# AwesomePeiweiPan/Droid-SLAM_Reserch

Measured on AMD Instinct MI355X. Metric: BA update iters/sec (2000-edge equivalents; 256 keyframes, 48x64), higher is better.
Workload: dtype f32; 1 GPU; 256-keyframe / 2000-edge global BA, 48x64, t0=1, lm=1e-5 ep=1e-2 (BASELINE configs[2]); edges_total=2000, solve=fp64 dense Cholesky on device, chol_failed=False

## Files before the change

droid-slam_reserch_amd/csrc/api.hip:

```cpp
#include <hip/hip_runtime.h>
#include <stdarg.h>
#include <stdio.h>

#include <map>
#include <mutex>

#include "../../include/droid_backends_hip.h"
#include "../../include/droid_test_hooks_hip.h"
#include "../../include/droid_heads_hip.h"
#include "../../include/droid_motion_encode_hip.h"
#include "../../include/droid_update_hip.h"
#include "ba_internal.hpp"
#include "graph.hpp"
#include "launchers.hpp"

using namespace droid;

static thread_local char g_err[512] = "";

static std::map<const void*, int*> g_mirror;
static std::mutex g_mirror_mu;
struct HintState { int* ptr; int tag; };
static std::map<const void*, HintState> g_hint;
static int g_hint_tag = 0;
static void hints_of(BaView& v, const void* ws, bool new_call) {
  std::lock_guard<std::mutex> lock(g_mirror_mu);
  auto it = g_hint.find(ws);
  if (it == g_hint.end()) return;
  if (new_call) it->second.tag = g_hint_tag = g_hint_tag >= (1 << 30) ? 1 : g_hint_tag + 1;
  if (it->second.tag == 0) return;
  v.hint = it->second.ptr;
  v.hint_tag = it->second.tag;
}
static int* mirror_of(const void* ws) {
  std::lock_guard<std::mutex> lock(g_mirror_mu);
  auto it = g_mirror.find(ws);
  return it == g_mirror.end() ? nullptr : it->second;
}

static int fail(int code, const char* fmt, ...) {
  va_list ap;
  va_start(ap, fmt);
  vsnprintf(g_err, sizeof(g_err), fmt, ap);
  va_end(ap);
  return code;
}

static int fail_hip(const char* where, hipError_t e) {
  return e == hipSuccess ? DROID_OK : fail(DROID_E_HIP, "%s: %s", where, hipGetErrorString(e));
}

static int check_hip(const char* where) { return fail_hip(where, hipGetLastError()); }

static bool bytes_overlap(const void* p, uint64_t p_bytes, const void* q, uint64_t q_bytes) {
  const uintptr_t a = (uintptr_t)p, b = (uintptr_t)q;
  const uintptr_t a1 = a + (p_bytes > UINTPTR_MAX - a ? UINTPTR_MAX - a : p_bytes);
  const uintptr_t b1 = b + (q_bytes > UINTPTR_MAX - b ? UINTPTR_MAX - b : q_bytes);
  return p_bytes > 0 && q_bytes > 0 && a < b1 && b < a1;
}
static uint64_t f32_bytes(uint64_t elems) { return elems > UINT64_MAX / 4 ? UINT64_MAX : elems * 4; }

// ... 434 lines not shown
  if (hints) {
    hints[0] = hints[1] = 0;
    g_hint[workspace] = HintState{hints, 0};
  }
  else g_hint.erase(workspace);
  return DROID_OK;
}

int droid_ba_attach_status_mirror(const void* workspace, int* mirror) {
  if (!workspace) return fail(DROID_E_ARG, "ba_attach_status_mirror: null %s", "workspace");
  std::lock_guard<std::mutex> lock(g_mirror_mu);
  if (mirror) g_mirror[workspace] = mirror;
  else g_mirror.erase(workspace);
  return DROID_OK;
}

int droid_test_wave_reduce32(const float* in, float* out, void* stream) {
  if (!in || !out) return fail(DROID_E_ARG, "test_wave_reduce32: null %s", "pointer");
  launch_wave_reduce32_test(in, out, (hipStream_t)stream);
  return check_hip("test_wave_reduce32");
}

int droid_test_ba_lin(const float* poses, const float* disps, const float* intrinsics, const float* disps_sens,
                      const float* targets, const float* weights, const float* eta, const int64_t* ii, const int64_t* jj,
                      int E, int nbuf, int H, int W, int M, int t0, int t1, int motion_only, int ragged, void* workspace,
                      size_t workspace_bytes, float* hpart_out, float* q_out, float* w_out, float* ebuf_out,
                      size_t* words_out, void* stream) {
  const BaDims d{E, nbuf, H, W, M, t0, t1, motion_only};
  BaView v;
  if (int rc = ba_view(v, workspace, workspace_bytes, d)) return rc;
  if (!poses || !disps || !intrinsics) return fail(DROID_E_ARG, "test_ba_lin: null %s", "state pointer");
  if (E > 0 && (!targets || !weights || !ii || !jj)) return fail(DROID_E_ARG, "test_ba_lin: null %s", "edge data");
  if (!motion_only && v.M > 0 && (!eta || !disps_sens)) return fail(DROID_E_ARG, "test_ba_lin: null %s", "eta/disps_sens");
  hipStream_t s = (hipStream_t)stream;
  const size_t words[4] = {(size_t)E * v.nch * LIN_WAVES * 32, (size_t)v.M * v.HW, (size_t)v.M * v.HW,
                           v.wide ? 6 * ((size_t)v.M + E) * v.HW : 0};
  const float* src[4] = {v.Hpart, v.Q, v.w, v.Ebuf};
  float* dst[4] = {hpart_out, q_out, w_out, ebuf_out};
  if (dst[0] || dst[1] || dst[2] || dst[3])
    launch_lin_test(v, poses, disps, intrinsics, disps_sens, targets, weights, eta, ii, jj, motion_only != 0, ragged != 0, s);
  if (words_out) {
    words_out[4] = (size_t)v.wide;
    words_out[5] = (size_t)v.zsplit;
  }
  for (int k = 0; k < 4; k++) {
    if (words_out) words_out[k] = words[k];
    if (dst[k] && words[k])
      (void)hipMemcpyAsync(dst[k], src[k], sizeof(float) * words[k], hipMemcpyDeviceToDevice, s);
  }
  return check_hip("test_ba_lin");
}

size_t droid_chol_scratch_doubles(int n) { return CholSystem::scratch_doubles(n); }

int droid_chol_solve(const double* A, const double* b, double* x, int n, double* scratch,
                     int* fail_flag, void* stream) {
  if (n <= 0 || !A || !b || !x || !scratch || !fail_flag) return fail(DROID_E_ARG, "chol_solve: bad %s", "argument");
  hipStream_t s = (hipStream_t)stream;
  const CholSystem c(scratch, n, x, fail_flag);
  launch_chol_pack(A, b, c.S, c.n, c.ld, s);
  launch_chol_solve(c, 0.0, 0.0, s, false);
  return check_hip("chol_solve");
}

int droid_frame_distance(const float* poses, const float* disps, const float* intrinsics,
                         const int64_t* ii, const int64_t* jj, int E, int nbuf, int H, int W,
                         float beta, float* dist, void* stream) {
  if (E < 0 || nbuf <= 0 || H <= 0 || W <= 0) return fail(DROID_E_ARG, "frame_distance: bad %s", "sizes");
  if (E == 0) return DROID_OK;
  if (!poses || !disps || !intrinsics || !ii || !jj || !dist) return fail(DROID_E_ARG, "frame_distance: null %s", "pointer");
  launch_frame_distance(poses, disps, intrinsics, ii, jj, E, nbuf, H, W, beta, dist, (hipStream_t)stream);
  return check_hip("frame_distance");
}

int droid_frame_distance_matrix(const float* poses, const float* disps, const float* intrinsics, int n, int nbuf,
                                int H, int W, float beta, float* dist, void* stream) {
  if (n < 0 || nbuf <= 0 || n > nbuf || H <= 0 || W <= 0) return fail(DROID_E_ARG, "frame_distance_matrix: bad %s", "sizes");
  if (n == 0) return DROID_OK;
  if (!poses || !disps || !intrinsics || !dist) return fail(DROID_E_ARG, "frame_distance_matrix: null %s", "pointer");
  launch_frame_distance_matrix(poses, disps, intrinsics, n, H, W, beta, dist, (hipStream_t)stream);
  return check_hip("frame_distance_matrix");
}

int droid_projmap(const float* poses, const float* disps, const float* intrinsics,
                  const int64_t* ii, const int64_t* jj, int E, int nbuf, int H, int W,
                  float* coords, float* valid, void* stream) {
  if (E < 0 || nbuf <= 0 || H <= 0 || W <= 0) return fail(DROID_E_ARG, "projmap: bad %s", "sizes");
  if (E == 0) return DROID_OK;
  if (!poses || !disps || !intrinsics || !ii || !jj || !coords || !valid) return fail(DROID_E_ARG, "projmap: null %s", "pointer");
  launch_projmap(poses, disps, intrinsics, ii, jj, E, nbuf, H, W, coords, valid, (hipStream_t)stream);
  return check_hip("projmap");
}

int droid_reproject_motion(const float* poses, const float* disps, const float* intrinsics, int intr_stride,
                           const int64_t* ii, const int64_t* jj, const float* target, int E, int nbuf, int H, int W,
                           float* coords, float* valid, float* motn, void* stream) {
  if (E < 0 || nbuf <= 0 || H <= 0 || W <= 0 || (intr_stride != 0 && intr_stride != 4))
    return fail(DROID_E_ARG, "reproject_motion: bad %s", "sizes");
  if (E == 0) return DROID_OK;
  if (!poses || !disps || !intrinsics || !ii || !jj || !coords || !valid) return fail(DROID_E_ARG, "reproject_motion: null %s", "pointer");
  if (motn && !target) return fail(DROID_E_ARG, "reproject_motion: motn needs %s", "target");
  launch_reproject_motion(poses, disps, intrinsics, intr_stride, ii, jj, target, E, nbuf, H, W, coords, valid, motn,
                          (hipStream_t)stream);
  return check_hip("reproject_motion");
}

// ... 374 lines not shown
```

droid-slam_reserch_amd/csrc/ba_internal.hpp:

```cpp
#pragma once
#include <hip/hip_runtime.h>
#include <stddef.h>
#include <stdint.h>

namespace droid {

constexpr int LIN_THREADS = 256;
constexpr int LIN_PPT = 2;
constexpr int LIN_CP = LIN_THREADS * LIN_PPT;
constexpr int LIN_WAVES = LIN_THREADS / 64;
constexpr int CHOL_NB = 64;
__host__ __device__ inline int chol_ld(int n) { return (n + 1 + 15) & ~15; }
__host__ __device__ inline size_t chol_flag_words(int n) { return 2 * ((size_t)(n + 1 + CHOL_NB - 1) / CHOL_NB) + 8; }
__host__ __device__ inline int chol_tile_index(int nrb, int bi, int bj) { return bj * nrb - bj * (bj - 1) / 2 + (bi - bj); }
__host__ __device__ inline size_t chol_tiles(int n) {
  const int nb = (n + CHOL_NB - 1) / CHOL_NB, nrb = (n + 1 + CHOL_NB - 1) / CHOL_NB;
  return (size_t)chol_tile_index(nrb, nb, nb);
}
__host__ __device__ inline size_t chol_mbuf_offset(int n) { return ((size_t)(n + CHOL_NB - 1) / CHOL_NB) * CHOL_NB * CHOL_NB; }
__host__ __device__ inline size_t chol_lfin_offset(int n) { return 2 * chol_mbuf_offset(n); }
__host__ __device__ inline size_t chol_ldiag_doubles(int n) { return chol_lfin_offset(n) + chol_tiles(n) * CHOL_NB * CHOL_NB; }
__host__ __device__ inline int chol_bs_pairs_grid(int nb) { return (nb + 1) / 2; }
__host__ __device__ inline int chol_bs_pairs_owner(int col) { return col / 2; }
__host__ __device__ inline int chol_bs_pairs_first(int wg) { return 2 * wg; }

__host__ __device__ inline size_t pk_colbase(int n, int J) {
  return (size_t)CHOL_NB * ((size_t)J * (size_t)(n + 1) - (size_t)CHOL_NB * (size_t)J * (size_t)(J - 1) / 2);
}
__host__ __device__ inline int pk_width(int n, int J) { return (n - CHOL_NB * J) < CHOL_NB ? (n - CHOL_NB * J) : CHOL_NB; }
__host__ __device__ inline size_t pk_total(int n) {
  if (n <= 0) return 0;
  const int nb = (n + CHOL_NB - 1) / CHOL_NB;
  return pk_colbase(n, nb - 1) + (size_t)(n + 1 - CHOL_NB * (nb - 1)) * (size_t)pk_width(n, nb - 1);
}
__host__ __device__ inline size_t pk_index(int n, int gi, int gj) {
  const int J = gj / CHOL_NB;
  return pk_colbase(n, J) + (size_t)(gi - CHOL_NB * J) * (size_t)pk_width(n, J) + (size_t)(gj - CHOL_NB * J);
}
__host__ __device__ inline unsigned pk_index32(int n, int gi, int gj) {
  const int J = gj >> 6, c0 = J << 6;
  const int w = (n - c0) < CHOL_NB ? (n - c0) : CHOL_NB;
  return (unsigned)(CHOL_NB * (J * (n + 1) - (CHOL_NB / 2) * J * (J - 1)) + (gi - c0) * w + (gj - c0));
}

enum { HDR_STATUS = 0, HDR_M = 1, HDR_CHOL_FAIL = 2, HDR_NENT = 3, HDR_NWORK = 4,
       HDR_NC1 = 5, HDR_NC2 = 6,
       HDR_WORDS = 16 };
enum { STATUS_BAD_INDEX = 1, STATUS_ETA_ROWS = 2, STATUS_CHOL_FAIL = 4, STATUS_CHOL_STALL = 8 };

struct BaView {
  int E, nbuf, H, W, HW;
  int t0, t1, P, M;
  int n, ld;
  int nch;
  int own0, own1;
  int motion_only;
  int* hdr;
  int* slot_of;
  int* kx;
  int* seg_ptr;
  int* seg_edge;
  int* cursor;
  int* ent_ptr;
  int* ent_row;
  int* ent_pose;
  int* wk_ptr;
  int* order;
  int* xtmp;
  int* cls_list;
  int* gt_ptr;
  double* Gpart;
  int s2_split;
  float* Hpart;
  float* Q;
// ... 89 lines not shown
  v.Gpart = nullptr;
  if (M > 0) {
    const int ptiles = (v.HW + 63) / 64;
    int ns = S2_WGS / M;
    v.s2_split = ns < 1 ? 1 : (ns > ptiles ? ptiles : ns);
    size_t tiles = (size_t)E * 7 / 4 + (size_t)M + 1;
    if (tiles > (size_t)28 * M) tiles = (size_t)28 * M;
    v.Gpart = static_cast<double*>(take(sizeof(double) * (tiles * v.s2_split * 256 + 64)));
  }
  v.sys = static_cast<double*>(take(sizeof(double) * ((size_t)(v.n + 1) * v.ld + 8)));
  v.psys = static_cast<double*>(take(sizeof(double) * (pk_total(v.n) + 8)));
  v.packed = 0;
  v.xsol = static_cast<double*>(take(sizeof(double) * ((size_t)v.ld + 1)));
  v.bs_flags = static_cast<int*>(take(sizeof(int) * chol_flag_words(v.n)));
  v.ldiag = static_cast<double*>(take(sizeof(double) * chol_ldiag_doubles(v.n)));
  v.dx = static_cast<float*>(take(sizeof(float) * ((size_t)v.n + 8)));
  v.ov_ready = static_cast<int*>(take(sizeof(int) * ((size_t)(v.n + 1 + CHOL_NB - 1) / CHOL_NB + 8)));
  v.pose_snap = static_cast<float*>(take(sizeof(float) * 7 * (size_t)nbuf));
  return off;
}

__host__ __device__ inline int solver_preset_words(const BaView& v) {
  return (int)((reinterpret_cast<const char*>(v.bs_flags) - reinterpret_cast<const char*>(v.xsol)) / 4 +
               (long)chol_flag_words(v.n));
}
__host__ __device__ inline int solver_preset_tiles(const BaView& v) { return v.n > 0 ? (int)chol_tiles(v.n) : 0; }

struct BaLaunchPlan {
  int zero_wgs;
  int asm_units;
  dim3 schur2;
  int sf_split;
  dim3 syrk[2], fold;
};
inline BaLaunchPlan ba_launch_plan(const BaView& v) {
  BaLaunchPlan p;
  p.zero_wgs = LIN_ZERO_WGS;
  p.asm_units = v.E > 0 ? v.E + (solver_preset_words(v) + 1023) / 1024 + solver_preset_tiles(v) : 0;
  p.schur2 = dim3(v.M + (p.asm_units + 4 * v.s2_split - 1) / (4 * v.s2_split), v.s2_split);
  const int tiles = (v.HW + SF_TP - 1) / SF_TP, ns = SF_WGS / (v.M > 0 ? v.M : 1);
  p.sf_split = ns < 1 ? 1 : (ns > tiles ? tiles : ns);
  p.syrk[0] = dim3(v.M, v.sy_ns[0], 1);
  p.syrk[1] = dim3(v.M, v.sy_ns[1], 4);
  p.fold = dim3(v.M, SY_FOLD_GROUPS, 2);
  return p;
}

struct CholSystem {
  double* S; int n, ld; double* x; int* flags; double* ldiag; int* fail;
  explicit CholSystem(const BaView& v)
      : S(v.sys), n(v.n), ld(v.ld), x(v.xsol), flags(v.bs_flags), ldiag(v.ldiag), fail(v.hdr + HDR_CHOL_FAIL) {}
  CholSystem(double* scratch, int n, double* x, int* fail);
  static size_t scratch_doubles(int n);
};

void launch_wave_reduce32_test(const float* in, float* out, hipStream_t s);
void launch_lin_test(const BaView& v, const float* poses, const float* disps, const float* intr, const float* sens,
                     const float* targets, const float* weights, const float* eta, const int64_t* ii, const int64_t* jj,
                     bool motion_only, bool ragged, hipStream_t s);
void launch_prep(const BaView& v, const int64_t* ii, const int64_t* jj, hipStream_t s);
void launch_unpack_system(const BaView& v, hipStream_t s);
void launch_build_stage(const BaView& v, const BaLaunchPlan& plan, const float* poses, const float* disps,
                        const float* intr, const float* sens, const float* targets, const float* weights,
                        const float* eta, const int64_t* ii, const int64_t* jj, bool motion_only,
                        int stage, hipStream_t s);
void launch_update(const BaView& v, float* poses, float* disps, const float* intr, const float* weights,
                   const int64_t* ii, const int64_t* jj, const double* x, float* dx_out, float* dz_out,
                   bool motion_only, hipStream_t s, int* status_mirror = nullptr);
void launch_chol_preset(const CholSystem& c, hipStream_t s);
bool launch_chol_factor(const CholSystem& c, double lm, double ep, hipStream_t s);
void launch_chol_backsolve(const CholSystem& c, bool factor_single, hipStream_t s);
void launch_chol_solve(const CholSystem& c, double lm, double ep, hipStream_t s, bool preset_done);

void launch_unpack_cols(const BaView& v, int J0, int J1, double lm, double ep, int epoch, hipStream_t s);
bool launch_chol_factor_overlap(const CholSystem& c, const int* ready, int epoch, hipStream_t s);
bool chol_overlap_available(int n);

}
```

droid-slam_reserch_amd/csrc/chol.hip:

```cpp
#include <hip/hip_runtime.h>
#include <mutex>

#include <cstdint>
#include <cstdlib>

#include "ba_internal.hpp"
#include "launchers.hpp"

namespace droid {

constexpr int NB = CHOL_NB;

#ifdef CHOL_STAMPS
__device__ unsigned long long g_chol_stamps[64 * 16];
__device__ unsigned long long g_bs_stamps[64 * 8];
__shared__ unsigned long long g_chol_lstamps[16];
extern "C" int droid_debug_chol_stamps(unsigned long long* out) {
  return (int)hipMemcpyFromSymbol(out, HIP_SYMBOL(g_chol_stamps), sizeof(unsigned long long) * 64 * 16);
}
extern "C" int droid_debug_bs_stamps(unsigned long long* out) {
  return (int)hipMemcpyFromSymbol(out, HIP_SYMBOL(g_bs_stamps), sizeof(unsigned long long) * 64 * 8);
}
#define STEP_STAMP(slot)                                                                                      \
  do { if (threadIdx.x == 0 && panel && (blockIdx.x < 2))                                                      \
// ... 583 lines not shown
      if (wave < nd) {
        const int q = p + 1 + wave;
        wave_gemm_nt16<true>(&B2[(16 * q) * LDP + 16 * p], &B2[(16 * q) * LDP + 16 * p], &Wl[WLB * p], WLP);
      } else if (solve_rows && wave < nd + 4) {
        const int g = wave - nd;
        wave_gemm_nt16<true>(&BT[(16 * g) * LDP + 16 * p], &BT[(16 * g) * LDP + 16 * p], &Wl[WLB * p], WLP);
      }
    }
    if (p == 0) TILE_STAMP(10);
    __syncthreads();
    if (p == 0) TILE_STAMP(5);
    if (PERSIST && solve_rows && wave == 4)
      chol_strip_out(S, ld, lfin_slot(Ldiag, n, bi, kp), BT, r0, c0, wk, nrows, p, (p == 3) ? &done[bi] : nullptr,
                     4 * kp + 3);
    if (p == 3) break;
    const int q = p + 1;
    if (wave == 0) {
      wave_gemm_nt16<false>(&B2[(16 * q) * LDP + 16 * q], &B2[(16 * q) * LDP + 16 * p],
                            &B2[(16 * q) * LDP + 16 * p], LDP);
      wave_potrf16(&B2[(16 * q) * LDP + 16 * q], &Wl[WLB * q], Idn, fail, diag);
      if (p == 0) TILE_STAMP(6);
    } else {
      int cnt = 0;
#pragma unroll 1
      for (int r = q; r < 4; r++)
#pragma unroll 1
        for (int s2 = q; s2 <= r; s2++) {
          if (r == q && s2 == q) continue;
          {
            const int slot = cnt % 2;
            const int owner = 1 + slot + ((1 + slot >= q) ? 1 : 0);
            if (owner == wave)
              wave_gemm_nt16<false>(&B2[(16 * r) * LDP + 16 * s2], &B2[(16 * r) * LDP + 16 * p],
                                    &B2[(16 * s2) * LDP + 16 * p], LDP);
          }
          cnt++;
        }
      const bool mine = (wave >= 5) ? (ndef > 0) : (ndef > 0 && wave == q);
      if (mine) {
        f64x4 acc = dacc[0];
        if (!PERSIST && k >= 0) strip_update_tile(acc, B0, B1, dg, q);
#pragma unroll
        for (int pp = 0; pp < 3; pp++)
          if (pp <= p) block_update16(acc, &BT[(16 * dg) * LDP + 16 * pp], &B2[(16 * q) * LDP + 16 * pp]);
        store_solve(acc, dg, q);
        dacc[0] = dacc[1];
        dacc[1] = dacc[2];
      }
    }
    __syncthreads();
    if (p == 0) TILE_STAMP(7);
  }
  TILE_STAMP(8);
  if (PERSIST && bi == kp + 1 && kp + 1 < (n + NB - 1) / NB) {
    __syncthreads();
    if (wave < 4) {
      const int g = wave;
#pragma unroll
      for (int q = 3; q >= 0; q--) {
        lds_f64* Cq = &BT[(16 * g) * LDP + 16 * q];
        f64x4 acc;
#pragma unroll
        for (int i = 0; i < 4; i++) acc[i] = Cq[(fg + 4 * i) * LDP + fr];
#pragma unroll
        for (int s2 = q + 1; s2 < 4; s2++)
#pragma unroll
          for (int kk = 0; kk < 16; kk += 4)
            acc = __builtin_amdgcn_mfma_f64_16x16x4f64(-BT[(16 * g + fr) * LDP + 16 * s2 + kk + fg],
                                                       B2[(16 * s2 + kk + fg) * LDP + 16 * q + fr], acc, 0, 0, 0);
#pragma unroll
        for (int i = 0; i < 4; i++) Cq[(fg + 4 * i) * LDP + fr] = acc[i];
        f64x4 m = {0.0, 0.0, 0.0, 0.0};
#pragma unroll
        for (int kk = 0; kk < 16; kk += 4)
          m = __builtin_amdgcn_mfma_f64_16x16x4f64(Cq[fr * LDP + kk + fg], Wl[WLB * q + (kk + fg) * WLP + fr], m, 0, 0, 0);
#pragma unroll
        for (int i = 0; i < 4; i++) Cq[(fg + 4 * i) * LDP + fr] = m[i];
      }
      gbl_f64* Mj = Ldiag + chol_mbuf_offset(n) + (size_t)kp * NB * NB;
#pragma unroll
      for (int it = 0; it < 8; it++) {
        const int u = it * 64 + lane;
        const int i = 16 * g + (u >> 5), j2 = (u & 31) * 2;
        f64x2 v = *(const lds_f64x2*)&BT[i * LDP + j2];
        if (r0 + i >= n) v = (f64x2){0.0, 0.0};
        *(gbl_f64x2*)&Mj[i * NB + j2] = v;
      }
    }
  }
  if (PERSIST && diag) {
#pragma unroll
    for (int e = t; e < 1024; e += 512) {
      const int pb = e >> 8, j = (e >> 4) & 15, kk = e & 15;
      const int br = pb == 3 ? 1 : 0, bc = pb == 3 ? 2 : pb + 1;
      B2[(16 * br + j) * LDP + 16 * bc + kk] = Wl[WLB * pb + WLP * j + kk];
    }
    __syncthreads();
  }
  if (grp == 0) {
    if (diag) {
      if (PERSIST) store_tile64(Ldiag + (size_t)kp * NB * NB, B2, NB, 0, 0, 0, NB, NB, false);
      else store_tile64(S, B2, ld, c0, c0, c0, c0 + wk, wk, true);
    }
  } else if (solve_rows && !PERSIST) {
    store_tile64(S, BT, ld, r0, c0, max(r0, c0 + wk), min(r0 + NB, nrows), wk, false);
  }
  if (!PERSIST) TILE_STAMP(9);
}

__global__ __launch_bounds__(512) void chol_step_kernel(double* __restrict__ S, int n, int ld, int k,
                                                        int* __restrict__ fail, double lm, double ep) {
  chol_tile<false>((gbl_f64*)S, n, ld, k, k + 1 + (int)blockIdx.x, k + 1 + (int)blockIdx.y, fail, lm, ep, nullptr,
                   nullptr, nullptr);
}


template <bool OV>
__device__ __attribute__((noinline)) void chol_tile_persist(double* __restrict__ S, int n, int ld, int k, int bi,
                                                            int bj, int* __restrict__ fail, double lm, double ep,
                                                            double* __restrict__ Ldiag, int* __restrict__ done,
                                                            int* __restrict__ abortf, bool coh_first, int k_last) {
  chol_tile<true, OV>((gbl_f64*)S, n, ld, k, bi, bj, fail, lm, ep, (gbl_f64*)Ldiag, done, abortf, coh_first, k_last);
}

struct CfpInput { const int* flag; int need; const gbl_f64* slot; };
__device__ __forceinline__ bool cfp_waits_for_done(int bj, int k, bool panel) { return k >= 0 && !panel && bj != k + 2; }
__device__ __forceinline__ int cfp_first_step(int bj) { return (bj == 0) ? -1 : 0; }
template <bool OV>
__device__ __forceinline__ CfpInput cfp_input(int lane, int bi, int bj, int k, bool panel, const int* done,
                                              const int* dver, const int* ready, int epoch, double* Ldiag, int n) {
  const bool flagged = cfp_waits_for_done(bj, k, panel);
  CfpInput in = {nullptr, 4 * k + 3, nullptr};
// ... 384 lines not shown
    if (B > 0 && rowb < B) {                                                                           \
      double u0 = 0.0, u1 = 0.0;                                                                       \
      _Pragma("unroll") for (int ii = 0; ii < 16; ii += 2) {                                           \
        const f64x2 xx = *(const lds_f64x2*)&DROID_LDS(xk)[16 * B + ii];                                \
        u0 = fma(Lcol[16 * B + ii], xx[0], u0);                                                        \
        u1 = fma(Lcol[16 * B + ii + 1], xx[1], u1);                                                    \
      }                                                                                                \
      z -= u0 + u1;                                                                                    \
    }
    DROID_BS_BLOCK(3)
    DROID_BS_BLOCK(2)
    DROID_BS_BLOCK(1)
    DROID_BS_BLOCK(0)
#undef DROID_BS_BLOCK
#undef DROID_BS_WTERM
#undef DROID_BS_STEP
    BS_STAMP(2);
    if (FAST && j < nb - 1) xsol -= poll_matvec(j + 1, Mc);
    if (__double_as_longlong(xsol) == BSP_SENTINEL) xsol = __longlong_as_double(0x7ff8000000000000LL);
    BS_STAMP(4);
    if (t < wj) __hip_atomic_store(&x[c0 + t], xsol, __ATOMIC_RELAXED, __HIP_MEMORY_SCOPE_AGENT);
    BS_STAMP(5);
  }
}

#ifdef CHOL_STAMPS
#define BS_STAMP_W(slot, wv) do { if (threadIdx.x == 64 * (wv) && blockIdx.x < 64) g_bs_stamps[blockIdx.x * 8 + (slot)] = wall_clock64(); } while (0)
#else
#define BS_STAMP_W(slot, wv) do { } while (0)
#endif

struct BspTileRegs { f64x2 v[4]; };
__device__ __forceinline__ BspTileRegs bsp_tile_issue(const gbl_f64* __restrict__ src, size_t pitch, int rows_valid) {
  const int t = threadIdx.x;
  BspTileRegs r;
#pragma unroll
  for (int it = 0; it < 4; it++) {
    const int idx2 = it * 512 + t, i = idx2 >> 5, j = (idx2 & 31) * 2;
    const bool ok = i < rows_valid;
    r.v[it] = *(const gbl_f64x2*)(src + (ok ? (size_t)i * pitch + j : 0));
    if (!ok) r.v[it] = (f64x2){0.0, 0.0};
  }
  return r;
}
__device__ __forceinline__ void bsp_tile_store(lds_f64* __restrict__ dst, const BspTileRegs& r) {
  const int t = threadIdx.x;
#pragma unroll
  for (int it = 0; it < 4; it++) {
    const int idx2 = it * 512 + t, i = idx2 >> 5, j = (idx2 & 31) * 2;
    *(lds_f64x2*)(&dst[i * LDP + j]) = r.v[it];
  }
}

constexpr int BSP_DC = 10 * 256;
__device__ __forceinline__ int bsp_dc_source(int e) {
  const int blk = e >> 7, i = (e & 127) >> 3, j = (e & 7) * 2;
  int br, bc;
  if (blk < 6) {
    br = blk < 1 ? 1 : (blk < 3 ? 2 : 3);
    bc = blk - br * (br - 1) / 2;
  } else {
    br = blk == 9 ? 1 : 0;
    bc = blk == 9 ? 2 : blk - 5;
  }
  return (16 * br + i) * NB + 16 * bc + j;
}

__device__ __forceinline__ void bsp_times_inverse(lds_f64* T, const lds_f64* D, int g, int lane) {
  const int fr = lane & 15, fg = lane >> 4;
#pragma unroll
  for (int q = 3; q >= 0; q--) {
    lds_f64* Cq = &T[(16 * g) * LDP + 16 * q];
    f64x4 acc;
#pragma unroll
    for (int i = 0; i < 4; i++) acc[i] = Cq[(fg + 4 * i) * LDP + fr];
#pragma unroll
    for (int s2 = q + 1; s2 < 4; s2++)
#pragma unroll
      for (int kk = 0; kk < 16; kk += 4)
        acc = __builtin_amdgcn_mfma_f64_16x16x4f64(-T[(16 * g + fr) * LDP + 16 * s2 + kk + fg],
                                                   D[(s2 * (s2 - 1) / 2 + q) * 256 + (kk + fg) * 16 + fr], acc, 0, 0, 0);
#pragma unroll
    for (int i = 0; i < 4; i++) Cq[(fg + 4 * i) * LDP + fr] = acc[i];
    f64x4 m = {0.0, 0.0, 0.0, 0.0};
#pragma unroll
    for (int kk = 0; kk < 16; kk += 4)
      m = __builtin_amdgcn_mfma_f64_16x16x4f64(Cq[fr * LDP + kk + fg], D[(6 + q) * 256 + (kk + fg) * 16 + fr], m, 0, 0, 0);
#pragma unroll
    for (int i = 0; i < 4; i++) Cq[(fg + 4 * i) * LDP + fr] = m[i];
  }
}

template <int NN>
__device__ __forceinline__ double bsp_dot(const double* col, const lds_f64* xs) {
  double a0 = 0.0, a1 = 0.0, a2 = 0.0, a3 = 0.0;
#pragma unroll
  for (int r = 0; r < NN; r += 4) {
    const f64x2 x01 = *(const lds_f64x2*)&xs[r], x23 = *(const lds_f64x2*)&xs[r + 2];
    a0 = fma(col[r + 0], x01[0], a0);
    a1 = fma(col[r + 1], x01[1], a1);
    a2 = fma(col[r + 2], x23[0], a2);
    a3 = fma(col[r + 3], x23[1], a3);
  }
  return (a0 + a1) + (a2 + a3);
}

__global__ __launch_bounds__(512) void chol_backsolve_pairs_kernel(
    double* __restrict__ S_, int n, int ld, double* __restrict__ x, int* __restrict__ err,
    const double* __restrict__ Ldiag_) {
  __shared__ double Dc[2][BSP_DC];
  __shared__ double Nt[3][NB * LDP];
  __shared__ double xs[8][NB];
  __shared__ double far_part[8][NB];
  __shared__ double near_part[8][NB];
  __shared__ double us[2][NB];
  __shared__ int dead;
  const gbl_f64* const S = (const gbl_f64*)S_;
  const gbl_f64* const Ldiag = (const gbl_f64*)Ldiag_;
  const int t = threadIdx.x, w = t >> 6, l = t & 63;
  const int nb = (n + NB - 1) / NB, G = gridDim.x, J = blockIdx.x;
  const int b = chol_bs_pairs_first(J), a = b + 1;
  const bool has_a = a < nb;
  const bool above = a + 1 < nb;
  const bool above2 = a + 2 < nb;
  const int ch = w & 1, rq = w >> 1;
  lds_f64* const xw = DROID_LDS(xs[w]);
  BS_STAMP_W(0, 0);
  if (t == 0) dead = 0;

  const int ra = (a + 1) * NB, rb = (a + 2) * NB;
  BspTileRegs t0, t1, t2;
  f64x2 dreg[5];
  if (above) {
    t1 = bsp_tile_issue(S + (size_t)ra * ld + (size_t)b * NB, ld, n - ra);
    if (above2) {
      t2 = bsp_tile_issue(S + (size_t)rb * ld + (size_t)b * NB, ld, n - rb);
      t0 = bsp_tile_issue(S + (size_t)rb * ld + (size_t)a * NB, ld, n - rb);
    }
#pragma unroll
    for (int it = 0; it < 5; it++) {
      const int idx2 = it * 512 + t, which = idx2 >= BSP_DC / 2 ? 1 : 0;
      dreg[it] = *(const gbl_f64x2*)(Ldiag + (size_t)(b + which) * NB * NB + bsp_dc_source(idx2 - which * (BSP_DC / 2)));
    }
  }

  double keep[NB];
  {
    const gbl_f64* base = Ldiag;
    int row_lo = 0, col_lo = l, row_hi = 0, used = 0;
    if (w == 4 || (w == 5 && has_a)) {
      const int pb = l >> 4;
      base = Ldiag + (size_t)(b + w - 4) * NB * NB;
      row_lo = pb == 3 ? 16 : 0;
      col_lo = 16 * (pb == 3 ? 2 : pb + 1) + (l & 15);
      used = NB;
    } else if (w == 6 && has_a) {
      base = Ldiag + chol_mbuf_offset(n) + (size_t)b * NB * NB;
      used = NB;
    } else if (ch == 1 && rq < 2 && above) {
      base = Ldiag + chol_mbuf_offset(n) + (size_t)a * NB * NB;
      row_lo = row_hi = 32 * rq;
      used = 32;
    }
#pragma unroll
    for (int i = 0; i < NB; i++) {
      keep[i] = 0.0;
      if (i < used) keep[i] = base[(size_t)((i < 16 ? row_lo : row_hi) + i) * NB + (i < 16 ? col_lo : l)];
    }
  }
  double z = 0.0;
  if ((w == 4 || (w == 5 && has_a)) && (b + w - 4) * NB + l < n) z = S[(size_t)n * ld + (b + w - 4) * NB + l];

  if (above) {
    bsp_tile_store(DROID_LDS(Nt[1]), t1);
    if (above2) {
      bsp_tile_store(DROID_LDS(Nt[2]), t2);
      bsp_tile_store(DROID_LDS(Nt[0]), t0);
    }
#pragma unroll
    for (int it = 0; it < 5; it++) *(lds_f64x2*)&DROID_LDS(Dc[0])[2 * (it * 512 + t)] = dreg[it];
    __syncthreads();
    if (w < 4) {
      bsp_times_inverse(DROID_LDS(Nt[1]), DROID_LDS(Dc[0]), w, l);
      if (above2) bsp_times_inverse(DROID_LDS(Nt[0]), DROID_LDS(Dc[1]), w, l);
    } else if (above2) {
      bsp_times_inverse(DROID_LDS(Nt[2]), DROID_LDS(Dc[0]), w - 4, l);
    }
  }
  BS_STAMP_W(1, 0);

  auto poll = [&](int gi, int lanes) -> double {
    double xv = 0.0;
    if (l < lanes && gi + l < n) {
      int spins = 0;
      while (true) {
        xv = __hip_atomic_load(&x[gi + l], __ATOMIC_RELAXED, __HIP_MEMORY_SCOPE_AGENT);
        if (__double_as_longlong(xv) != BSP_SENTINEL) break;
        if (++spins > (1 << 22)) {
          *(volatile int*)&dead = 1;
          atomicMax(err, 2);
          xv = 0.0;
          break;
        }
        __builtin_amdgcn_s_sleep(1);
      }
    }
    return xv;
  };

  double far = 0.0;
  for (int P = G - 1; P >= J + 2; P--) {
    if (*(volatile int*)&dead) break;
    const int r0 = 2 * P * NB + 32 * rq;
    const gbl_f64* col = S + (size_t)(b + ch) * NB + l;
    double Tc[32];
#pragma unroll
    for (int r = 0; r < 32; r++) {
      const int row = r0 + r;
      Tc[r] = col[(size_t)(row < n ? row : n - 1) * ld];
      if (row >= n) Tc[r] = 0.0;
    }
    const double xv = poll(r0, 32);
    if (l < 32) xw[l] = xv;
    far += bsp_dot<32>(Tc, xw);
  }
  DROID_LDS(far_part[w])[l] = far;
  BS_STAMP_W(2, 0);
  __syncthreads();
  if (dead) return;

  if (w == 4 || (w == 5 && has_a)) {
    const int c = w - 4;
    z -= (far_part[c][l] + far_part[2 + c][l]) + (far_part[4 + c][l] + far_part[6 + c][l]);
    const int rowb = l >> 4;
    double xsol = 0.0;
#define DROID_BSP_WTERM(ACC, C)                                                                         \
    asm volatile("v_fmac_f64_dpp %0, %1, %2 row_newbcast:" #C " row_mask:0xf bank_mask:0xf"             \
                 : "+v"(ACC) : "v"(z), "v"(keep[C]));
#define DROID_BSP_BLOCK(B)                                                                              \
    if (rowb == B) {                                                                                   \
// ... 183 lines not shown
  return false;
}

extern "C" int droid_debug_bs_pairs_map(int nb, int* owner) {
  for (int j = 0; j < nb; j++) owner[j] = chol_bs_pairs_owner(j);
  return chol_bs_pairs_grid(nb);
}

void launch_chol_backsolve(const CholSystem& c, bool factor_single, hipStream_t s) {
  const int nb = (c.n + NB - 1) / NB;
  if (nb >= 2 && nb <= BSP_MAX_BLOCKS) {
    CholSystem a = c;
    const double* ld_arg = factor_single ? c.ldiag : nullptr;
    void* args[] = {&a.S, &a.n, &a.ld, &a.x, &a.fail, &ld_arg};
    const bool pairs = factor_single && chol_switches().bs_pairs;
    const void* fn = pairs ? (const void*)chol_backsolve_pairs_kernel
                   : factor_single ? (const void*)chol_backsolve_persistent_kernel<true>
                                   : (const void*)chol_backsolve_persistent_kernel<false>;
    if (launch_spinning_grid(fn, pairs ? chol_bs_pairs_grid(nb) : nb, pairs ? 512 : 256, args, s,
                             chol_switches().force_bs_refusal)) return;
  }
  if (factor_single)
    hipLaunchKernelGGL(chol_ldiag_to_sys_kernel, dim3(nb), dim3(256), 0, s, c.S, c.n, c.ld, c.ldiag);
  for (int k = nb - 1; k >= 0; k--) {
    const int c0 = k * NB;
    hipLaunchKernelGGL(chol_backsolve_kernel, dim3(1 + (c0 + 255) / 256), dim3(256), 0, s, c.S, c.n,
                       c.ld, k, c.x);
  }
}

void launch_chol_preset(const CholSystem& c, hipStream_t s) {
  (void)hipMemsetAsync(c.fail, 0, sizeof(int), s);
  const size_t xbytes = sizeof(double) * (size_t)c.n, fbytes = sizeof(int) * chol_flag_words(c.n);
  const char* xb = reinterpret_cast<const char*>(c.x);
  const char* fb = reinterpret_cast<const char*>(c.flags);
  if (fb >= xb + xbytes && fb - xb <= (ptrdiff_t)(xbytes + 4096)) {
    (void)hipMemsetAsync(c.x, 0xFF, (size_t)(fb - xb) + fbytes, s);
  } else {
    (void)hipMemsetAsync(c.x, 0xFF, xbytes, s);
    (void)hipMemsetAsync(c.flags, 0xFF, fbytes, s);
  }
  (void)hipMemsetAsync(c.ldiag + chol_lfin_offset(c.n), 0xFF, sizeof(double) * chol_tiles(c.n) * NB * NB, s);
}

void launch_chol_solve(const CholSystem& c, double lm, double ep, hipStream_t s, bool preset_done) {
  if (c.n <= 0) return;
  if (!preset_done) launch_chol_preset(c, s);
  const bool single = launch_chol_factor(c, lm, ep, s);
  launch_chol_backsolve(c, single, s);
}

size_t CholSystem::scratch_doubles(int n) {
  if (n <= 0) return 0;
  return (size_t)(n + 1) * chol_ld(n) + chol_ldiag_doubles(n) + (chol_flag_words(n) + 1) / 2 + 16;
}
CholSystem::CholSystem(double* scratch, int n_, double* x_, int* fail_)
    : S(scratch), n(n_), ld(chol_ld(n_)), x(x_), fail(fail_) {
  ldiag = S + (size_t)(n + 1) * ld;
  flags = reinterpret_cast<int*>(ldiag + chol_ldiag_doubles(n));
}

__global__ void chol_pack_kernel(const double* __restrict__ A, const double* __restrict__ b,
                                 double* __restrict__ S, int n, int ld) {
  const size_t idx = (size_t)blockIdx.x * blockDim.x + threadIdx.x;
  if (idx >= (size_t)(n + 1) * ld) return;
  const int r = (int)(idx / ld), c = (int)(idx % ld);
  double val = 0.0;
  if (r < n && c < n) val = A[(size_t)r * n + c];
  else if (r == n && c < n) val = b[c];
  S[idx] = val;
}

void launch_chol_pack(const double* A, const double* b, double* S, int n, int ld, hipStream_t s) {
  const size_t tot = (size_t)(n + 1) * ld;
  hipLaunchKernelGGL(chol_pack_kernel, dim3((unsigned)((tot + 255) / 256)), dim3(256), 0, s, A, b,
                     S, n, ld);
}

}
```

droid-slam_reserch_amd/droid_backends/_lib.py:

```python
from __future__ import annotations

import ctypes
import os

_HERE = os.path.dirname(os.path.abspath(__file__))
LIB_PATH = os.environ.get("DROID_HIP_LIB") or os.path.join(_HERE, "libdroid_backends_hip.so")

ABI = {
    "droid_abi_version": ("i", ""),
    "droid_last_error": ("s", ""),
    "droid_corr_index_forward": ("i", "3p 7i p"),
    "droid_corr_index_backward": ("i", "3p 7i p"),
    "droid_corr_pyramid_forward": ("i", "P 2p 6i p"),
    "droid_corr_volume_pyramid": ("i", "3p P 7i 2l i p"),
    "droid_corr_pyramid_forward_slots": ("i", "P 3p i l 5i p"),
    "droid_corr_volume_pyramid_slots": ("i", "3p P p 7i l i p"),
    "droid_altcorr_forward": ("i", "4p 9i p"),
    "droid_altcorr_backward": ("i", "6p 8i p"),
    "droid_altcorr_pyramid_forward": ("i", "P 4p 7i p"),
    "droid_altcorr_pyramid_forward_f16": ("i", "P 4p 7i p"),
    "droid_ba_workspace_bytes": ("z", "7i"),
    "droid_ba": ("i", "9p 8i 2f i 3p z p"),
    "droid_ba_prepare": ("i", "2p 10i p z p"),
    "droid_ba_build": ("i", "9p 8i p z p"),
# ... 5 lines not shown
    "droid_ba_unpack_chunk": ("i", "9i 2f i p z p"),
    "droid_ba_solve_update_overlap": ("i", "6p 9i 3p z p"),
    "droid_ba_solve_update": ("i", "6p 7i 2f i 3p z p"),
    "droid_ba_profile_iteration": ("i", "9p 7i 2f i p z 2p"),
    "droid_ba_system": ("p", "p 7i Z"),
    "droid_ba_status": ("i", "2p 2I"),
    "droid_ba_attach_status_mirror": ("i", "2p"),
    "droid_ba_attach_launch_hints": ("i", "2p"),
    "droid_chol_solve": ("i", "3p i 3p"),
    "droid_chol_scratch_doubles": ("z", "i"),
    "droid_reproject_motion": ("i", "3p i 3p 4i 4p"),
    "droid_frame_distance": ("i", "5p 4i f 2p"),
    "droid_frame_distance_matrix": ("i", "3p 4i f 2p"),
    "droid_projmap": ("i", "5p 4i 3p"),
    "droid_iproj": ("i", "3p 3i 2p"),
    "droid_depth_filter": ("i", "5p 4i 2p"),
    "droid_proximity_workspace_bytes": ("z", "5i"),
    "droid_proximity_edges": ("i", "p 7i f 2i 2p i 2p i p i 2p z p"),
    "droid_cvx_upsample": ("i", "4p 6i p"),
    "droid_graph_mean_workspace_bytes": ("z", "2i"),
    "droid_graph_mean": ("i", "3p i l 4i 2p z p"),
    "droid_se3_unary": ("i", "2p l i p"),
    "droid_se3_mul": ("i", "p i p i p l p"),
    "droid_pose_interpolate": ("i", "2p i p i 4p"),
    "droid_point_cloud_workspace_bytes": ("z", "3i"),
    "droid_point_cloud": ("i", "6p 5i d 6p z p"),
    "droid_test_wave_reduce32": ("i", "3p"),
}
SYMBOLS = list(ABI)
ABI_UPDATE = {
    "droid_ba_inputs_workspace_bytes": ("z", "3i"),
    "droid_ba_inputs": ("i", "11p 9i f 6p i 3p i 2p z p"),
}
SYMBOLS_UPDATE = list(ABI_UPDATE)
ABI_CORR_ENCODE = {
    "droid_corr_encode_packed_bytes": ("z", ""),
    "droid_corr_encode": ("i", "P 4p i l 7i p"),
}
SYMBOLS_CORR_ENCODE = list(ABI_CORR_ENCODE)
ABI_MOTION_ENCODE = {
    "droid_motion_encode_packed_bytes": ("z", ""),
    "droid_motion_encode": ("i", "3p i 8p 5i p"),
}
SYMBOLS_MOTION_ENCODE = list(ABI_MOTION_ENCODE)
ABI_HEADS = {
    "droid_head_packed_bytes": ("z", "i"),
    "droid_update_heads": ("i", "3P 2I 5i p"),
}
SYMBOLS_HEADS = list(ABI_HEADS)
ABI_TEST = {
    "droid_test_ba_lin": ("i", "9p 9i p z 4p Z p"),
}
SYMBOLS_TEST = list(ABI_TEST)
_CTYPE = {"i": ctypes.c_int, "l": ctypes.c_int64, "z": ctypes.c_size_t, "f": ctypes.c_float, "d": ctypes.c_double,
          "p": ctypes.c_void_p, "P": ctypes.POINTER(ctypes.c_void_p), "I": ctypes.POINTER(ctypes.c_int),
          "Z": ctypes.POINTER(ctypes.c_size_t), "s": ctypes.c_char_p}


def signature(name):
    for table in (ABI, ABI_TEST, ABI_CORR_ENCODE, ABI_MOTION_ENCODE, ABI_HEADS):
        if name in table:
            break
    else:
        table = ABI_UPDATE
    res, args = table[name]
    return _CTYPE[res], [_CTYPE[run[-1]] for run in args.split() for _ in range(int(run[:-1] or 1))]


DROID_F16, DROID_F32, DROID_F64 = 0, 1, 2

_lib = None


class DroidBackendError(RuntimeError):
    pass


def load() -> ctypes.CDLL:
    global _lib
    if _lib is not None:
        return _lib
    if not os.path.exists(LIB_PATH):
        raise DroidBackendError(
            f"{LIB_PATH} is missing: build the HIP extension first "
            "(python -c 'import __graft_entry__ as g; g.build()' or droid-slam_reserch_amd/csrc/build.sh). "
            "There is no CPU fallback.")
    lib = ctypes.CDLL(LIB_PATH)
    for s in SYMBOLS + SYMBOLS_UPDATE + SYMBOLS_CORR_ENCODE + SYMBOLS_MOTION_ENCODE + SYMBOLS_HEADS + SYMBOLS_TEST:
        if not hasattr(lib, s):
            if s in SYMBOLS_TEST:
                continue
            raise DroidBackendError(f"{LIB_PATH} does not export {s}")
        fn = getattr(lib, s)
        fn.restype, fn.argtypes = signature(s)
    if lib.droid_abi_version() != 1:
        raise DroidBackendError("ABI version mismatch")
    _lib = lib
    return lib


def check(rc: int, what: str):
    if rc != 0:
        msg = load().droid_last_error().decode("utf-8", "replace")
        raise RuntimeError(f"droid_backends.{what} failed (rc={rc}): {msg}")
```

Baseline: 2086 iters/s.

## Precompute inverse-scaled off-diagonal tiles in factor for pair backsolve

The factor kernel now also writes the inverse-scaled sub-diagonal tiles for blocks two and three below the panel into new scratch buffers (N2, N3). The pair backsolve kernel loads those precomputed tiles directly. This drops its own loads of the diagonal-inverse blocks and the LDS triangular multiply by the inverse. The cost is extra scratch memory and extra MFMA work and stores in the factor tail, plus a test hook that exposes the scratch layout.

```diff
diff --git a/droid-slam_reserch_amd/csrc/api.hip b/droid-slam_reserch_amd/csrc/api.hip
--- a/droid-slam_reserch_amd/csrc/api.hip
+++ b/droid-slam_reserch_amd/csrc/api.hip
@@ -7,6 +7,7 @@
 
 #include "../../include/droid_backends_hip.h"
 #include "../../include/droid_test_hooks_hip.h"
+#include "../../include/droid_chol_hooks_hip.h"
 #include "../../include/droid_heads_hip.h"
 #include "../../include/droid_motion_encode_hip.h"
 #include "../../include/droid_update_hip.h"
@@ -547,6 +548,18 @@
 }
 
 size_t droid_chol_scratch_doubles(int n) { return CholSystem::scratch_doubles(n); }
+
+int droid_test_chol_layout(int n, int64_t* out) {
+  if (n <= 0 || !out) return fail(DROID_E_ARG, "test_chol_layout: bad %s", "argument");
+  const size_t ldiag = CholSystem::scratch_ldiag(n);
+  out[0] = chol_ld(n);
+  out[1] = (int64_t)ldiag;
+  out[2] = (int64_t)(ldiag + chol_mbuf_offset(n));
+  out[3] = (int64_t)(ldiag + chol_n2_offset(n));
+  out[4] = (int64_t)(ldiag + chol_n3_offset(n));
+  out[5] = (n + CHOL_NB - 1) / CHOL_NB;
+  return DROID_OK;
+}
 
 int droid_chol_solve(const double* A, const double* b, double* x, int n, double* scratch,
                      int* fail_flag, void* stream) {
diff --git a/droid-slam_reserch_amd/csrc/ba_internal.hpp b/droid-slam_reserch_amd/csrc/ba_internal.hpp
--- a/droid-slam_reserch_amd/csrc/ba_internal.hpp
+++ b/droid-slam_reserch_amd/csrc/ba_internal.hpp
@@ -19,7 +19,9 @@
 }
 __host__ __device__ inline size_t chol_mbuf_offset(int n) { return ((size_t)(n + CHOL_NB - 1) / CHOL_NB) * CHOL_NB * CHOL_NB; }
 __host__ __device__ inline size_t chol_lfin_offset(int n) { return 2 * chol_mbuf_offset(n); }
-__host__ __device__ inline size_t chol_ldiag_doubles(int n) { return chol_lfin_offset(n) + chol_tiles(n) * CHOL_NB * CHOL_NB; }
+__host__ __device__ inline size_t chol_n2_offset(int n) { return chol_lfin_offset(n) + chol_tiles(n) * CHOL_NB * CHOL_NB; }
+__host__ __device__ inline size_t chol_n3_offset(int n) { return chol_n2_offset(n) + chol_mbuf_offset(n); }
+__host__ __device__ inline size_t chol_ldiag_doubles(int n) { return chol_n3_offset(n) + chol_mbuf_offset(n); }
 __host__ __device__ inline int chol_bs_pairs_grid(int nb) { return (nb + 1) / 2; }
 __host__ __device__ inline int chol_bs_pairs_owner(int col) { return col / 2; }
 __host__ __device__ inline int chol_bs_pairs_first(int wg) { return 2 * wg; }
@@ -215,6 +217,7 @@
       : S(v.sys), n(v.n), ld(v.ld), x(v.xsol), flags(v.bs_flags), ldiag(v.ldiag), fail(v.hdr + HDR_CHOL_FAIL) {}
   CholSystem(double* scratch, int n, double* x, int* fail);
   static size_t scratch_doubles(int n);
+  static size_t scratch_ldiag(int n);
 };
 
 void launch_wave_reduce32_test(const float* in, float* out, hipStream_t s);
diff --git a/droid-slam_reserch_amd/csrc/chol.hip b/droid-slam_reserch_amd/csrc/chol.hip
--- a/droid-slam_reserch_amd/csrc/chol.hip
+++ b/droid-slam_reserch_amd/csrc/chol.hip
@@ -659,7 +659,10 @@
     if (p == 0) TILE_STAMP(7);
   }
   TILE_STAMP(8);
-  if (PERSIST && bi == kp + 1 && kp + 1 < (n + NB - 1) / NB) {
+  const int below = bi - kp;
+  const bool leaves_n = PERSIST && bi < (n + NB - 1) / NB &&
+                        (below == 1 || below == 2 || (below == 3 && chol_bs_pairs_first(chol_bs_pairs_owner(kp)) == kp));
+  if (leaves_n) {
     __syncthreads();
     if (wave < 4) {
       const int g = wave;
@@ -684,7 +687,8 @@
 #pragma unroll
         for (int i = 0; i < 4; i++) Cq[(fg + 4 * i) * LDP + fr] = m[i];
       }
-      gbl_f64* Mj = Ldiag + chol_mbuf_offset(n) + (size_t)kp * NB * NB;
+      gbl_f64* Mj = Ldiag + (below == 1 ? chol_mbuf_offset(n) : below == 2 ? chol_n2_offset(n) : chol_n3_offset(n)) +
+                    (size_t)kp * NB * NB;
 #pragma unroll
       for (int it = 0; it < 8; it++) {
         const int u = it * 64 + lane;
@@ -1175,45 +1179,6 @@
   }
 }
 
-constexpr int BSP_DC = 10 * 256;
-__device__ __forceinline__ int bsp_dc_source(int e) {
-  const int blk = e >> 7, i = (e & 127) >> 3, j = (e & 7) * 2;
-  int br, bc;
-  if (blk < 6) {
-    br = blk < 1 ? 1 : (blk < 3 ? 2 : 3);
-    bc = blk - br * (br - 1) / 2;
-  } else {
-    br = blk == 9 ? 1 : 0;
-    bc = blk == 9 ? 2 : blk - 5;
-  }
-  return (16 * br + i) * NB + 16 * bc + j;
-}
-
-__device__ __forceinline__ void bsp_times_inverse(lds_f64* T, const lds_f64* D, int g, int lane) {
-  const int fr = lane & 15, fg = lane >> 4;
-#pragma unroll
-  for (int q = 3; q >= 0; q--) {
-    lds_f64* Cq = &T[(16 * g) * LDP + 16 * q];
-    f64x4 acc;
-#pragma unroll
-    for (int i = 0; i < 4; i++) acc[i] = Cq[(fg + 4 * i) * LDP + fr];
-#pragma unroll
-    for (int s2 = q + 1; s2 < 4; s2++)
-#pragma unroll
-      for (int kk = 0; kk < 16; kk += 4)
-        acc = __builtin_amdgcn_mfma_f64_16x16x4f64(-T[(16 * g + fr) * LDP + 16 * s2 + kk + fg],
-                                                   D[(s2 * (s2 - 1) / 2 + q) * 256 + (kk + fg) * 16 + fr], acc, 0, 0, 0);
-#pragma unroll
-    for (int i = 0; i < 4; i++) Cq[(fg + 4 * i) * LDP + fr] = acc[i];
-    f64x4 m = {0.0, 0.0, 0.0, 0.0};
-#pragma unroll
-    for (int kk = 0; kk < 16; kk += 4)
-      m = __builtin_amdgcn_mfma_f64_16x16x4f64(Cq[fr * LDP + kk + fg], D[(6 + q) * 256 + (kk + fg) * 16 + fr], m, 0, 0, 0);
-#pragma unroll
-    for (int i = 0; i < 4; i++) Cq[(fg + 4 * i) * LDP + fr] = m[i];
-  }
-}
-
 template <int NN>
 __device__ __forceinline__ double bsp_dot(const double* col, const lds_f64* xs) {
   double a0 = 0.0, a1 = 0.0, a2 = 0.0, a3 = 0.0;
@@ -1231,7 +1196,6 @@
 __global__ __launch_bounds__(512) void chol_backsolve_pairs_kernel(
     double* __restrict__ S_, int n, int ld, double* __restrict__ x, int* __restrict__ err,
     const double* __restrict__ Ldiag_) {
-  __shared__ double Dc[2][BSP_DC];
   __shared__ double Nt[3][NB * LDP];
   __shared__ double xs[8][NB];
   __shared__ double far_part[8][NB];
@@ -1251,19 +1215,13 @@
   BS_STAMP_W(0, 0);
   if (t == 0) dead = 0;
 
-  const int ra = (a + 1) * NB, rb = (a + 2) * NB;
   BspTileRegs t0, t1, t2;
-  f64x2 dreg[5];
   if (above) {
-    t1 = bsp_tile_issue(S + (size_t)ra * ld + (size_t)b * NB, ld, n - ra);
+    const gbl_f64* N2 = Ldiag + chol_n2_offset(n);
+    t1 = bsp_tile_issue(N2 + (size_t)b * NB * NB, NB, NB);
     if (above2) {
-      t2 = bsp_tile_issue(S + (size_t)rb * ld + (size_t)b * NB, ld, n - rb);
-      t0 = bsp_tile_issue(S + (size_t)rb * ld + (size_t)a * NB, ld, n - rb);
-    }
-#pragma unroll
-    for (int it = 0; it < 5; it++) {
-      const int idx2 = it * 512 + t, which = idx2 >= BSP_DC / 2 ? 1 : 0;
-      dreg[it] = *(const gbl_f64x2*)(Ldiag + (size_t)(b + which) * NB * NB + bsp_dc_source(idx2 - which * (BSP_DC / 2)));
+      t2 = bsp_tile_issue(Ldiag + chol_n3_offset(n) + (size_t)b * NB * NB, NB, NB);
+      t0 = bsp_tile_issue(N2 + (size_t)a * NB * NB, NB, NB);
     }
   }
 
@@ -1300,15 +1258,7 @@
       bsp_tile_store(DROID_LDS(Nt[2]), t2);
       bsp_tile_store(DROID_LDS(Nt[0]), t0);
     }
-#pragma unroll
-    for (int it = 0; it < 5; it++) *(lds_f64x2*)&DROID_LDS(Dc[0])[2 * (it * 512 + t)] = dreg[it];
     __syncthreads();
-    if (w < 4) {
-      bsp_times_inverse(DROID_LDS(Nt[1]), DROID_LDS(Dc[0]), w, l);
-      if (above2) bsp_times_inverse(DROID_LDS(Nt[0]), DROID_LDS(Dc[1]), w, l);
-    } else if (above2) {
-      bsp_times_inverse(DROID_LDS(Nt[2]), DROID_LDS(Dc[0]), w - 4, l);
-    }
   }
   BS_STAMP_W(1, 0);
 
@@ -1598,11 +1548,12 @@
 
 size_t CholSystem::scratch_doubles(int n) {
   if (n <= 0) return 0;
-  return (size_t)(n + 1) * chol_ld(n) + chol_ldiag_doubles(n) + (chol_flag_words(n) + 1) / 2 + 16;
-}
+  return scratch_ldiag(n) + chol_ldiag_doubles(n) + (chol_flag_words(n) + 1) / 2 + 16;
+}
+size_t CholSystem::scratch_ldiag(int n) { return (size_t)(n + 1) * chol_ld(n); }
 CholSystem::CholSystem(double* scratch, int n_, double* x_, int* fail_)
     : S(scratch), n(n_), ld(chol_ld(n_)), x(x_), fail(fail_) {
-  ldiag = S + (size_t)(n + 1) * ld;
+  ldiag = S + scratch_ldiag(n);
   flags = reinterpret_cast<int*>(ldiag + chol_ldiag_doubles(n));
 }
 
diff --git a/droid-slam_reserch_amd/droid_backends/_lib.py b/droid-slam_reserch_amd/droid_backends/_lib.py
--- a/droid-slam_reserch_amd/droid_backends/_lib.py
+++ b/droid-slam_reserch_amd/droid_backends/_lib.py
@@ -81,13 +81,17 @@
     "droid_test_ba_lin": ("i", "9p 9i p z 4p Z p"),
 }
 SYMBOLS_TEST = list(ABI_TEST)
+ABI_TEST_CHOL = {
+    "droid_test_chol_layout": ("i", "i p"),
+}
+SYMBOLS_TEST_CHOL = list(ABI_TEST_CHOL)
 _CTYPE = {"i": ctypes.c_int, "l": ctypes.c_int64, "z": ctypes.c_size_t, "f": ctypes.c_float, "d": ctypes.c_double,
           "p": ctypes.c_void_p, "P": ctypes.POINTER(ctypes.c_void_p), "I": ctypes.POINTER(ctypes.c_int),
           "Z": ctypes.POINTER(ctypes.c_size_t), "s": ctypes.c_char_p}
 
 
 def signature(name):
-    for table in (ABI, ABI_TEST, ABI_CORR_ENCODE, ABI_MOTION_ENCODE, ABI_HEADS):
+    for table in (ABI, ABI_TEST, ABI_TEST_CHOL, ABI_CORR_ENCODE, ABI_MOTION_ENCODE, ABI_HEADS):
         if name in table:
             break
     else:
@@ -115,9 +119,10 @@
             "(python -c 'import __graft_entry__ as g; g.build()' or droid-slam_reserch_amd/csrc/build.sh). "
             "There is no CPU fallback.")
     lib = ctypes.CDLL(LIB_PATH)
-    for s in SYMBOLS + SYMBOLS_UPDATE + SYMBOLS_CORR_ENCODE + SYMBOLS_MOTION_ENCODE + SYMBOLS_HEADS + SYMBOLS_TEST:
+    for s in (SYMBOLS + SYMBOLS_UPDATE + SYMBOLS_CORR_ENCODE + SYMBOLS_MOTION_ENCODE + SYMBOLS_HEADS + SYMBOLS_TEST +
+              SYMBOLS_TEST_CHOL):
         if not hasattr(lib, s):
-            if s in SYMBOLS_TEST:
+            if s in SYMBOLS_TEST or s in SYMBOLS_TEST_CHOL:
                 continue
             raise DroidBackendError(f"{LIB_PATH} does not export {s}")
         fn = getattr(lib, s)
diff --git a/include/droid_chol_hooks_hip.h b/include/droid_chol_hooks_hip.h
--- /dev/null
+++ b/include/droid_chol_hooks_hip.h
@@ -0,0 +1,15 @@
+#ifndef DROID_CHOL_HOOKS_HIP_H
+#define DROID_CHOL_HOOKS_HIP_H
+
+#include "droid_backends_hip.h"
+
+#ifdef __cplusplus
+extern "C" {
+#endif
+
+int droid_test_chol_layout(int n, int64_t *out);
+
+#ifdef __cplusplus
+}
+#endif
+#endif
```

Result: no change. 2101 iters/s (median of 6 runs) (+0.7%).
